# Weepingchestnut/SAVSR

Hardware: AMD Instinct MI355X
Metric: HR Mpixels/sec (Vid4-shape x4, 7-frame window) (higher is better)
Workload: dtype f32 (bf16x3 split products, fp32 accumulate)

## Files before the change

### savsr_amd/csrc/conv_common.hpp

```cpp
#pragma once
#include "common.hpp"

namespace savsr {

struct ConvParams {
    const float* src[SAVSR_MAX_SRC];
    int src_pix[SAVSR_MAX_SRC];
    const unsigned short* wimg;
    const float* bias;
    int act;
    float slope;
    const float* mul_px;
    const float* res1;
    int res1_pix;
    const float* res2;
    int res2_pix;
    float res2_scale;
    float* out;
    int out_pix;
    float* pool;
    int pool_stride;
};

#ifndef SAVSR_CONV_MAX_BATCH
#define SAVSR_CONV_MAX_BATCH 24
#endif
constexpr int CONV_MAX_BATCH = SAVSR_CONV_MAX_BATCH;
constexpr int CONV_WIDE_MIN_TILES = 200;
constexpr int CONV_WIDE_MIN_TILES_TP = 100;
#ifndef SAVSR_CONV_BLOCKS
#define SAVSR_CONV_BLOCKS 256
#endif
constexpr int CONV_PERSISTENT_BLOCKS = SAVSR_CONV_BLOCKS;
#ifndef WY_STRIP
#define WY_STRIP 1
#endif
struct MultiConvParams {
    ConvParams c[CONV_MAX_BATCH];
    int h, w, cout, nchunk, src_ch;
    int nconv, ncob, ntx, nty;
    int wy_tiles, wy_full, wy_strip_l2;
};
static_assert(sizeof(MultiConvParams) <= 4096, "MultiConvParams is passed by value as the conv kernels' argument: at most 4 KB");

int launch_conv_wy(const MultiConvParams& mp, hipStream_t st, bool f16);
int conv_wy_prepare_device();

typedef _Float16 f16x8 __attribute__((ext_vector_type(8)));
typedef _Float16 f16x4 __attribute__((ext_vector_type(4)));

#define SAVSR_GLOBAL __attribute__((address_space(1)))
__device__ __forceinline__ f32x4 ldg4(const float* base, unsigned byte_off) {
    return *(const SAVSR_GLOBAL f32x4*)((const SAVSR_GLOBAL char*)base + byte_off);
}
__device__ __forceinline__ float ldg1(const float* base, unsigned idx) {
    return *((const SAVSR_GLOBAL float*)base + idx);
}
#ifndef CONV_ST
#define CONV_ST 1
#endif
__device__ __forceinline__ void stg4(float* base, unsigned byte_off, const f32x4& v) {
#if CONV_ST == 1
    __builtin_nontemporal_store(v, (SAVSR_GLOBAL f32x4*)((SAVSR_GLOBAL char*)base + byte_off));
#else
    *(SAVSR_GLOBAL f32x4*)((SAVSR_GLOBAL char*)base + byte_off) = v;
#endif
}
__device__ __forceinline__ float vmax_raw(float a, float b) {
    float r;
    asm("v_max_f32 %0, %1, %2" : "=v"(r) : "v"(a), "v"(b));
    return r;
}
__device__ __forceinline__ void stg1(float* base, unsigned idx, float v) {
    *((SAVSR_GLOBAL float*)base + idx) = v;
}

}
```

### savsr_amd/csrc/conv_wy.hip

```cpp
#include "conv_common.hpp"

#include <type_traits>

#ifndef WY_STAMPS
#define WY_STAMPS 0
#endif
#ifndef WY_VALU
#define WY_VALU 6
#endif
#ifndef WY_FAST_EPILOGUE
#define WY_FAST_EPILOGUE 1
#endif
#ifndef WY_BUF
#define WY_BUF 1
#endif

namespace savsr {

namespace wy {
constexpr int TH = 16, TW = 32, NTHR = 512, COT = 64;
[[maybe_unused]] constexpr int IC = TW + 2;
#ifndef WY_ICP
#define WY_ICP 36
#endif
constexpr int ICP = WY_ICP;
constexpr int V_PLANE = 2 * ICP;
constexpr int V_WAVE = 2 * 2 * 2 * V_PLANE;
constexpr int W_HALF = 6 * 2 * 2 * 64;
constexpr int W_PHASE = 2 * W_HALF;
constexpr int EPS = 36;
constexpr int LDS_UNITS = 8 * V_WAVE + 2 * W_HALF;
constexpr size_t LDS_BYTES = 16ull * LDS_UNITS + 4ull * 8 * 32 * EPS;
static_assert(LDS_BYTES <= 160 * 1024, "LDS budget");
}

__device__ __attribute__((aligned(16))) const float g_wy_zero16[4] = {0.f, 0.f, 0.f, 0.f};

#if WY_STAMPS
__device__ long long g_wy_stamps[256 * 8 * 8];
#define WY_KSEC(i) (WY_STAMPS == 2 ? 0 : (i))
#define WY_MARK(i) do { const long long t_now = (long long)__builtin_amdgcn_s_memtime(); wy_sec[i] += t_now - wy_prev; wy_prev = t_now; } while (0)
#if WY_STAMPS == 2
#define WY_EMARK(i) WY_MARK(i)
#endif
#else
#define WY_KSEC(i) (i)
#define WY_MARK(i) do { } while (0)
#endif

typedef float f32x2 __attribute__((ext_vector_type(2)));
typedef __bf16 bf16x2 __attribute__((ext_vector_type(2)));
__device__ __forceinline__ void wy_split_store(const f32x4& v, bf16x4* hi_dst, bf16x4* lo_dst) {
    typedef unsigned u32x2 __attribute__((ext_vector_type(2)));
    const f32x2 a[2] = {{v[0], v[1]}, {v[2], v[3]}};
    u32x2 hi, lo;
#pragma unroll
    for (int p = 0; p < 2; ++p) hi[p] = __builtin_bit_cast(unsigned, __builtin_convertvector(a[p], bf16x2));
    asm("" : "+v"(hi[0]), "+v"(hi[1]));
#pragma unroll
    for (int p = 0; p < 2; ++p) {
        const f32x2 back = {__builtin_bit_cast(float, hi[p] << 16), __builtin_bit_cast(float, hi[p] & 0xffff0000u)};
        const f32x2 rest = {a[p][0] - back[0], a[p][1] - back[1]};
        lo[p] = __builtin_bit_cast(unsigned, __builtin_convertvector(rest, bf16x2));
    }
    *hi_dst = __builtin_bit_cast(bf16x4, hi);
    *lo_dst = __builtin_bit_cast(bf16x4, lo);
}
__device__ __forceinline__ void wy_f16_store(const f32x4& v, bf16x4* hi_dst) {
    f16x4 h;
#pragma unroll
    for (int j = 0; j < 4; ++j) h[j] = (_Float16)v[j];
    *hi_dst = __builtin_bit_cast(bf16x4, h);
}

template <bool FAST, bool F16>
__global__ __launch_bounds__(512) void conv_wy_kernel(const MultiConvParams mp) {
    using namespace wy;
    constexpr int WPH = F16 ? W_PHASE / 2 : W_PHASE, WHF = F16 ? W_HALF / 2 : W_HALF;
    extern __shared__ __attribute__((aligned(16))) unsigned char smem_raw[];
    bf16x8* smem = reinterpret_cast<bf16x8*>(smem_raw);
    const int tid = threadIdx.x, lane = tid & 63, wave = tid >> 6, half = lane >> 5, px = lane & 31;
    const int wave_s = __builtin_amdgcn_readfirstlane(wave);
    const int tiles_per_cob = mp.wy_tiles;
    const int total = mp.nconv * mp.ncob * tiles_per_cob;
    const int H = mp.h, W = mp.w;

    struct TileInfo { int conv, cob, x0, y0, tx, ty, strip; };
    auto decode = [&](int tile) {
        const int cc = (int)((unsigned)tile / (unsigned)tiles_per_cob), rem = tile - cc * tiles_per_cob;
        const bool strip = rem >= mp.wy_full;
        const int tyf = (int)((unsigned)rem / (unsigned)mp.ntx);
        const int l2 = strip ? mp.wy_strip_l2 : 3;
        const int ty = strip ? mp.nty - 1 : tyf;
        const int tx = strip ? (rem - mp.wy_full) << (3 - l2) : rem - tyf * mp.ntx;
        const int wx = tx + (wave_s >> l2);
        TileInfo ti;
        ti.conv = (int)((unsigned)cc / (unsigned)mp.ncob);
        ti.cob = cc - ti.conv * mp.ncob;
        ti.x0 = (wx < mp.ntx ? wx : tx) * TW;
        ti.y0 = wx < mp.ntx ? ty * TH - 2 * ((wave_s >> l2) << l2) : mp.nty * TH;
        ti.tx = tx;
        ti.ty = ty;
        ti.strip = strip ? 1 : 0;
        return ti;
    };

    f32x4 d[2][4], dx;
#if !WY_BUF
    int st_pxb[2], st_pxt;
    constexpr int INVALID = -(1 << 30);
#endif
    const float* st_base = nullptr;
    const bf16x8* st_w = nullptr;
    int st_pix = 0, st_cb = 0, st_src = 0, st_conv = 0, st_row0 = 0;
    const int q4 = lane & 3;
#if WY_BUF
    constexpr unsigned OOB = 0x80000000u;
    unsigned st_vcol[2], st_vtail;
    int st_x0 = 0;
    auto stage_cols = [&]() {
#pragma unroll
        for (int r = 0; r < 2; ++r) {
            const int x = st_x0 - 1 + (lane >> 2) + 16 * r;
            const unsigned v = (unsigned)(x * st_pix + 4 * q4) * 4u;
            st_vcol[r] = (unsigned)x < (unsigned)W ? v : OOB;
        }
        const int x = st_x0 - 1 + 32 + ((lane & 7) >> 2), rr = (lane >> 3) & 3, row = st_row0 + rr;
        const unsigned vt = (unsigned)((rr * W + x) * st_pix + 4 * q4) * 4u;
        const bool okt = (lane < 32) & ((unsigned)x < (unsigned)W) & ((unsigned)row < (unsigned)H);
        st_vtail = okt ? vt : OOB;
    };
#endif
#if WY_BUF
    auto uni = [](int v) { return __builtin_amdgcn_readfirstlane(v); };
    auto uni_ptr = [](const float* q) {
        const unsigned long long a = (unsigned long long)(uintptr_t)q;
        const unsigned lo = (unsigned)__builtin_amdgcn_readfirstlane((int)(unsigned)a), hi = (unsigned)__builtin_amdgcn_readfirstlane((int)(unsigned)(a >> 32));
        return (const float*)(uintptr_t)(((unsigned long long)hi << 32) | lo);
    };
#else
    auto uni = [](int v) { return v; };
    auto uni_ptr = [](const float* q) { return q; };
#endif
    auto stage_begin_tile = [&](const TileInfo& ti) {
        st_conv = ti.conv;
        st_src = 0;
        st_cb = 0;
        st_base = uni_ptr(mp.c[ti.conv].src[0]);
        st_pix = uni(mp.c[ti.conv].src_pix[0]);
        st_w = reinterpret_cast<const bf16x8*>(mp.c[ti.conv].wimg) + (long long)ti.cob * mp.nchunk * WPH;
        st_row0 = uni(ti.y0 + 2 * wave_s - 1);
#if WY_BUF
        st_x0 = ti.x0;
        stage_cols();
#else
#pragma unroll
        for (int r = 0; r < 2; ++r) {
            const int x = ti.x0 - 1 + (lane >> 2) + 16 * r;
            st_pxb[r] = (x >= 0 && x < W) ? st_row0 * W + x : INVALID;
        }
        {
            const int x = ti.x0 - 1 + 32 + ((lane & 7) >> 2), row = st_row0 + ((lane >> 3) & 3);
            st_pxt = (lane < 32 && x >= 0 && x < W && row >= 0 && row < H) ? row * W + x : INVALID;
        }
#endif
    };
    auto stage_advance = [&]() {
        st_cb += 16;
        st_w += WPH;
        if (st_cb >= mp.src_ch) {
            st_cb = 0;
            ++st_src;
            st_base = uni_ptr(mp.c[st_conv].src[st_src]);
#if WY_BUF
            const int pix_new = uni(mp.c[st_conv].src_pix[st_src]);
            if (pix_new != st_pix) { st_pix = pix_new; stage_cols(); }
#else
            st_pix = mp.c[st_conv].src_pix[st_src];
#endif
        }
    };
    int st_tile = blockIdx.x, st_chunk = 0;
    auto stage_next = [&]() -> bool {
        if (st_chunk + 1 < mp.nchunk) { ++st_chunk; stage_advance(); return true; }
        if (st_tile + (int)gridDim.x >= total) return false;
        st_tile += gridDim.x;
        st_chunk = 0;
        stage_begin_tile(decode(st_tile));
        return true;
    };
#if WY_BUF
    typedef unsigned u32x4_t __attribute__((ext_vector_type(4)));
    auto row_rsrc = [&](int i, bool whole) {
        const int off = ((st_row0 + i) * W * st_pix + st_cb) * 4;
        const bool row_ok = whole || (st_row0 + i >= 0 && st_row0 + i < H);
        return __builtin_amdgcn_make_buffer_rsrc((void*)((const char*)st_base + off), (short)0, row_ok ? 0x7fffffff : 0, 0x00020000);
    };
    auto issue_row = [&](int r, int i) {
        d[r][i] = __builtin_bit_cast(f32x4, (u32x4_t)__builtin_amdgcn_raw_buffer_load_b128(row_rsrc(i, false), (int)st_vcol[r], 0, 0));
    };
    auto issue_d = [&](int r) {
#pragma unroll
        for (int i = 0; i < 4; ++i) issue_row(r, i);
    };
    auto issue_dx = [&]() { dx = __builtin_bit_cast(f32x4, (u32x4_t)__builtin_amdgcn_raw_buffer_load_b128(row_rsrc(0, true), (int)st_vtail, 0, 0)); };
#else
    auto load_at = [&](int pixel, bool ok) -> f32x4 {
        const SAVSR_GLOBAL float* src = ok ? (const SAVSR_GLOBAL float*)st_base + (pixel * st_pix + st_cb + 4 * q4)
                                           : (const SAVSR_GLOBAL float*)g_wy_zero16;
        return *(const SAVSR_GLOBAL f32x4*)src;
    };
    auto issue_row = [&](int r, int i) {
        const bool row_ok = st_row0 + i >= 0 && st_row0 + i < H;
        d[r][i] = load_at(st_pxb[r] + i * W, row_ok && st_pxb[r] != INVALID);
    };
    auto issue_d = [&](int r) {
#pragma unroll
        for (int i = 0; i < 4; ++i) issue_row(r, i);
    };
    auto issue_dx = [&]() { dx = load_at(st_pxt, st_pxt != INVALID); };
#endif
    bf16x8* vwave = smem + wave * V_WAVE;
    constexpr int PLANE_B = V_PLANE * 16;
    const unsigned vst0 = (unsigned)(wave * V_WAVE + (q4 >> 1) * ICP + (lane >> 2)) * 16u + (unsigned)(q4 & 1) * 8u;
    const unsigned vst_t = (unsigned)(wave * V_WAVE + (q4 >> 1) * ICP + 32 + ((lane & 7) >> 2)) * 16u + (unsigned)(q4 & 1) * 8u;
    auto vptr = [&](unsigned off) { return reinterpret_cast<bf16x4*>(smem_raw + off); };
    auto vstore = [&](const f32x4& v, unsigned off) {
        if constexpr (F16) wy_f16_store(v, vptr(off));
        else wy_split_store(v, vptr(off), vptr(off + PLANE_B));
    };
    auto store_pair = [&](int r, int hf, const f32x4& va, const f32x4& vb) {
        vstore(va, vst0 + (unsigned)(r * 256 + (hf * 2 + 0) * 2 * PLANE_B));
        vstore(vb, vst0 + (unsigned)(r * 256 + (hf * 2 + 1) * 2 * PLANE_B));
    };
    auto store_one = [&](int r, int hf, int vr, const f32x4& v) {
        vstore(v, vst0 + (unsigned)(r * 256 + (hf * 2 + vr) * 2 * PLANE_B));
    };
    auto store_v0 = [&](int r) { store_one(r, 0, 0, d[r][0] - d[r][2]); };
    auto store_v1 = [&](int r) {
        store_one(r, 0, 1, d[r][1] + d[r][2]);
        const f32x4 v2 = d[r][2] - d[r][1], v3 = d[r][1] - d[r][3];
        d[r][0] = v2;
        d[r][1] = v3;
    };
    auto store_v01 = [&](int r) { store_v0(r); store_v1(r); };
    auto store_v23 = [&](int r) { store_pair(r, 1, d[r][0], d[r][1]); };
    const int grp = (lane >> 3) & 3;
    auto tail_value = [&](int hf) -> f32x4 {
        const int partner = hf == 0 ? (grp == 0 ? lane ^ 16 : lane ^ 24) : (grp == 2 ? lane ^ 24 : lane ^ 16);
        f32x4 o;
#pragma unroll
        for (int j = 0; j < 4; ++j) o[j] = __shfl(dx[j], partner, 64);
        return (hf == 0 && grp == 1) ? dx + o : dx - o;
    };
    auto tail_store = [&](int hf, const f32x4& v) {
        const bool mine = lane < 32 && (hf == 0 ? grp < 2 : (grp == 2 || grp == 1));
        const int vr = hf == 0 ? grp : (grp == 2 ? 0 : 1);
        if (mine) {
            vstore(v, vst_t + (unsigned)((hf * 2 + vr) * 2 * PLANE_B));
        }
    };
    auto store_vt01 = [&]() {
        const f32x4 v01 = tail_value(0), v23 = tail_value(1);
        tail_store(0, v01);
        dx = v23;
    };
    auto store_vt23 = [&]() { tail_store(1, dx); };
    bf16x8* wlds = smem + 8 * V_WAVE;
    [[maybe_unused]] const unsigned lane16 = (unsigned)lane * 16u;
    auto issue_w = [&](int j, int hf) {
        const int piece = F16 ? j * 8 + wave_s : wave_s * 3 + j;
        if (F16 && piece >= 12) return;
        const unsigned dst = __builtin_amdgcn_readfirstlane((unsigned)(uintptr_t)(wlds + hf * W_HALF + piece * (F16 ? 128 : 64)));
        unsigned keep;
#if WY_BUF
        asm volatile("s_mov_b32 %0, m0\n\ts_mov_b32 m0, %3\n\ts_nop 0\n\tglobal_load_lds_dwordx4 %1, %2\n\ts_mov_b32 m0, %0"
                     : "=&s"(keep) : "v"(lane16), "s"(st_w + hf * WHF + piece * 64), "s"(dst) : "memory");
#else
        asm volatile("s_mov_b32 %0, m0\n\ts_mov_b32 m0, %2\n\ts_nop 0\n\tglobal_load_lds_dwordx4 %1, off\n\ts_mov_b32 m0, %0"
                     : "=&s"(keep) : "v"(st_w + hf * WHF + piece * 64 + lane), "s"(dst) : "memory");
#endif
    };

    struct FragA { bf16x8 ah, al; };
    struct FragB { bf16x8 bh, bl; };
    const bf16x8* vrd = vwave + half * ICP + px;
    const bf16x8* wrd = wlds + lane;
    auto load_b = [&](int hf, int s, FragB& fr) {
        const int vr = s / 3, kx = s - 3 * vr;
        fr.bh = vrd[((hf * 2 + vr) * 2 + 0) * V_PLANE + kx];
        if (!F16) fr.bl = vrd[((hf * 2 + vr) * 2 + 1) * V_PLANE + kx];
    };
    auto load_a = [&](int hf, int s, int t, FragA& fr) {
        fr.ah = wrd[hf * W_HALF + ((s * 2 + t) * 2 + 0) * 64];
        if (!F16) fr.al = wrd[hf * W_HALF + ((s * 2 + t) * 2 + 1) * 64];
    };

    int tile = blockIdx.x;
#if WY_STAMPS
    long long wy_sec[8] = {0, 0, 0, 0, 0, 0, 0, 0};
    long long wy_prev = (long long)__builtin_amdgcn_s_memtime();
    const long long wy_t0 = wy_prev;
#endif
    FragA fa[2];
    FragB fb[2];
    if (tile < total) {
        stage_begin_tile(decode(tile));
#pragma unroll
        for (int j = 0; j < 3; ++j) issue_w(j, 0);
        issue_d(0);
        issue_d(1);
        issue_dx();
        store_v01(0);
        store_v01(1);
        store_vt01();
    }
    asm volatile("s_waitcnt vmcnt(0)" ::: "memory");
    __syncthreads();
    if (tile < total) { load_b(0, 0, fb[0]); load_a(0, 0, 0, fa[0]); }

    for (; tile < total; tile += gridDim.x) {
        const TileInfo cur = decode(tile);
        const ConvParams& p = mp.c[cur.conv];
        const int cob = cur.cob, x0 = cur.x0, y0 = cur.y0;
        f32x16 acc[4][2];
#pragma unroll
        for (int pz = 0; pz < 4; ++pz)
#pragma unroll
            for (int t = 0; t < 2; ++t)
#pragma unroll
                for (int i = 0; i < 16; ++i) acc[pz][t][i] = 0.f;
        const bool rows_in = y0 + 2 * wave_s < H;
        for (int chunk = 0; chunk < mp.nchunk; ++chunk) {
            auto phase = [&](auto mm) {
                constexpr bool MM = decltype(mm)::value;
                auto pieces = [&](int hf, int s) {
                    if (hf == 0) {
                        if (s == 0) { issue_w(0, 1); issue_w(1, 1); store_v23(0); }
                        if (s == 1) { issue_w(2, 1); stage_next(); issue_row(0, 0); }
                        if (s == 2) { store_v23(1); issue_row(0, 1); issue_row(0, 2); }
                        if (s == 3) { store_vt23(); issue_row(0, 3); issue_row(1, 0); }
                        if (s == 4) { issue_row(1, 1); issue_row(1, 2); }
                        if (s == 5) issue_row(1, 3);
                    } else {
                        if (s < 3) issue_w(s, 0);
                        if (s == 1) store_v0(0);
                        if (s == 2) store_v1(0);
                        if (s == 3) store_v0(1);
                        if (s == 4) store_v1(1);
                        if (s == 5) store_vt01();
                    }
                };
                auto mma3 = [&](int pz, int t, int sb) {
                    const FragA& a = fa[t];
                    const FragB& b = fb[sb];
                    if (MM && F16) {
                        acc[pz][t] = __builtin_amdgcn_mfma_f32_32x32x16_f16(__builtin_bit_cast(f16x8, a.ah), __builtin_bit_cast(f16x8, b.bh), acc[pz][t], 0, 0, 0);
                    } else if (MM) {
                        acc[pz][t] = __builtin_amdgcn_mfma_f32_32x32x16_bf16(a.al, b.bh, acc[pz][t], 0, 0, 0);
                        acc[pz][t] = __builtin_amdgcn_mfma_f32_32x32x16_bf16(a.ah, b.bl, acc[pz][t], 0, 0, 0);
                        acc[pz][t] = __builtin_amdgcn_mfma_f32_32x32x16_bf16(a.ah, b.bh, acc[pz][t], 0, 0, 0);
                    }
                };
#pragma unroll
                for (int hf = 0; hf < 2; ++hf) {
#pragma unroll
                    for (int s = 0; s < 5; ++s) {
                        const int pz = hf * 2 + s / 3;
                        load_a(hf, s, 1, fa[1]);
                        load_b(hf, s + 1, fb[(s + 1) & 1]);
                        __builtin_amdgcn_sched_barrier(0);
                        mma3(pz, 0, s & 1);
                        pieces(hf, s);
                        load_a(hf, s + 1, 0, fa[0]);
                        mma3(pz, 1, s & 1);
                        if (MM && F16) {
#pragma unroll
                            for (int i = 0; i < 2; ++i) {
                                __builtin_amdgcn_sched_group_barrier(0x008, 1, 0);
                                if (i == 1) __builtin_amdgcn_sched_group_barrier(0x100, 1, 0);
                                __builtin_amdgcn_sched_group_barrier(0x002, 3 * WY_VALU, 0);
                                __builtin_amdgcn_sched_group_barrier(0x200, 2, 0);
                                __builtin_amdgcn_sched_group_barrier(0x010, 1, 0);
                            }
                        } else if (MM) {
#pragma unroll
                            for (int i = 0; i < 6; ++i) {
                                __builtin_amdgcn_sched_group_barrier(0x008, 1, 0);
                                if (i == 3) __builtin_amdgcn_sched_group_barrier(0x100, 2, 0);
                                __builtin_amdgcn_sched_group_barrier(0x002, WY_VALU, 0);
                                __builtin_amdgcn_sched_group_barrier(0x200, 1, 0);
                                if (i == 1 || i == 4) __builtin_amdgcn_sched_group_barrier(0x010, 1, 0);
                            }
                        }
                        __builtin_amdgcn_sched_barrier(0);
                    }
                    {
                        const int pz = hf * 2 + 1;
                        load_a(hf, 5, 1, fa[1]);
                        __builtin_amdgcn_sched_barrier(0);
                        mma3(pz, 0, 1);
                        pieces(hf, 5);
                        if (MM) {
#pragma unroll
                            for (int i = 0; i < (F16 ? 1 : 3); ++i) {
                                __builtin_amdgcn_sched_group_barrier(0x008, 1, 0);
                                __builtin_amdgcn_sched_group_barrier(0x002, 10, 0);
                                __builtin_amdgcn_sched_group_barrier(0x200, 1, 0);
                            }
                        }
                        __builtin_amdgcn_sched_barrier(0);
                        WY_MARK(WY_KSEC(hf * 3 + 0));
                        if (hf == 0) asm volatile("s_waitcnt vmcnt(8)" ::: "memory");
                        else asm volatile("s_waitcnt vmcnt(0)" ::: "memory");
                        __syncthreads();
                        WY_MARK(WY_KSEC(hf * 3 + 1));
                        load_b(hf ^ 1, 0, fb[0]);
                        load_a(hf ^ 1, 0, 0, fa[0]);
                        __builtin_amdgcn_sched_barrier(0);
                        mma3(pz, 1, 1);
                        if (hf == 0) issue_dx();
                        __builtin_amdgcn_sched_barrier(0);
                    }
                    WY_MARK(WY_KSEC(hf * 3 + 2));
                }
            };
            auto phase_dead = [&]() {
#pragma unroll
                for (int j = 0; j < 3; ++j) issue_w(j, 1);
                stage_next();
                asm volatile("s_waitcnt vmcnt(0)" ::: "memory");
                __syncthreads();
#pragma unroll
                for (int j = 0; j < 3; ++j) issue_w(j, 0);
                asm volatile("s_waitcnt vmcnt(0)" ::: "memory");
                __syncthreads();
            };
            auto next_tile_rows_in = [&]() {
                if (tile + (int)gridDim.x >= total) return false;
                return decode(tile + (int)gridDim.x).y0 + 2 * wave_s < H;
            };
            if (rows_in) phase(std::true_type{});
            else if (chunk + 1 == mp.nchunk && next_tile_rows_in()) phase(std::false_type{});
            else phase_dead();
        }

        const float* e_bias = p.bias;
        const float* e_mul = p.mul_px;
        const float* e_r1 = p.res1;
        const float* e_r2 = p.res2;
        float* e_out = p.out;
        float* e_pool = p.pool;
        int e_act = p.act, e_opix = p.out_pix, e_r1pix = p.res1_pix, e_r2pix = p.res2_pix;
        float e_slope = p.slope, e_r2s = p.res2_scale;
        asm volatile("" : "+s"(e_bias), "+s"(e_mul), "+s"(e_r1), "+s"(e_r2), "+s"(e_out), "+s"(e_pool));
        asm volatile("" : "+s"(e_act), "+s"(e_opix), "+s"(e_r1pix), "+s"(e_r2pix), "+s"(e_slope), "+s"(e_r2s));
        const bool act_as_max = e_act == SAVSR_ACT_NONE || e_act == SAVSR_ACT_RELU || (e_act == SAVSR_ACT_LRELU && e_slope >= 0.f && e_slope <= 1.f);
        const float slope_eff = e_act == SAVSR_ACT_NONE ? 1.f : (e_act == SAVSR_ACT_RELU ? 0.f : e_slope);
        float* ep_base = reinterpret_cast<float*>(smem + LDS_UNITS);
        float* ep = ep_base + wave * (32 * EPS);
        const int c4 = lane & 7;
        const bool x_inside = x0 + TW <= W;
        const float* zero16 = (const float*)g_wy_zero16;
        const float* b_base = e_bias ? e_bias : zero16;
        const unsigned b_off = e_bias ? 4u * (unsigned)(cob * COT + 4 * c4) : 0u, b_step = e_bias ? 128u : 0u;
        f32x4 bias4[2];
#pragma unroll
        for (int t = 0; t < 2; ++t) bias4[t] = ldg4(b_base, b_off + (unsigned)t * b_step);
        const float* r1_base = e_r1 ? e_r1 : zero16;
        constexpr int RR = 2;
        f32x4 rr[RR][4];
        auto load_r1 = [&](int r, int t, f32x4 (&dst)[4]) {
            const int y = y0 + 2 * wave_s + r;
            const int co = cob * COT + 32 * t + 4 * c4;
            const unsigned off0 = 4u * (unsigned)((y * W + x0 + (lane >> 3)) * e_r1pix + co), ustride = 32u * (unsigned)e_r1pix;
            const bool row_ok = e_r1 && y < H;
#pragma unroll
            for (int i = 0; i < 4; ++i) {
                const bool ok = row_ok && (x_inside || x0 + (lane >> 3) + 8 * i < W);
                dst[i] = ldg4(r1_base, ok ? off0 + (unsigned)i * ustride : 0u);
            }
        };
#pragma unroll
        for (int gi = 0; gi < RR; ++gi) load_r1(gi / 2, gi % 2, rr[gi]);
        __builtin_amdgcn_sched_barrier(0);
#pragma unroll
        for (int t = 0; t < 2; ++t)
#pragma unroll
            for (int i = 0; i < 16; ++i) {
                const float m1 = acc[1][t][i], m2 = acc[2][t][i];
                acc[0][t][i] = (acc[0][t][i] + m1) + m2;
                acc[3][t][i] = (m1 - m2) - acc[3][t][i];
            }
        f32x4 psum[2][2];
#ifdef WY_EMARK
        asm volatile("" :: "v"(acc[0][0][0]), "v"(acc[3][1][15]));
        WY_EMARK(1);
#endif
#pragma unroll
        for (int r = 0; r < 2; ++r) {
            const int y = y0 + 2 * wave_s + r;
            const int pbase = y * W + x0 + (lane >> 3);
#pragma unroll
            for (int t = 0; t < 2; ++t) {
                psum[r][t] = f32x4{0.f, 0.f, 0.f, 0.f};
                const int gi = r * 2 + t;
                if (y >= H) {
                    asm volatile("" :: "v"(bias4[t]), "v"(rr[gi % RR][0]), "v"(rr[gi % RR][1]), "v"(rr[gi % RR][2]), "v"(rr[gi % RR][3]));
                    if (gi + RR < 4) load_r1((gi + RR) / 2, (gi + RR) % 2, rr[gi % RR]);
                    continue;
                }
                const f32x16& a = r == 0 ? acc[0][t] : acc[3][t];
#pragma unroll
                for (int g = 0; g < 4; ++g) {
                    const f32x4 v = {a[4 * g], a[4 * g + 1], a[4 * g + 2], a[4 * g + 3]};
                    *reinterpret_cast<f32x4*>(ep + px * EPS + 8 * g + 4 * half) = v;
                }
                const int co = cob * COT + 32 * t + 4 * c4;
                const f32x4 b4 = bias4[t];
                const unsigned ooff0 = 4u * (unsigned)(pbase * e_opix + co), ostride = 32u * (unsigned)e_opix;
                f32x4 ps = {0.f, 0.f, 0.f, 0.f};
#pragma unroll
                for (int ih = 0; ih < 2; ++ih) {
                    const int p0 = pbase + 16 * ih;
                    const bool ok0 = x_inside || x0 + (lane >> 3) + 16 * ih < W, ok1 = x_inside || x0 + (lane >> 3) + 16 * ih + 8 < W;
                    f32x4 v[2];
#pragma unroll
                    for (int i = 0; i < 2; ++i) {
                        const f32x4 a4 = *reinterpret_cast<const f32x4*>(ep + ((lane >> 3) + 16 * ih + 8 * i) * EPS + 4 * c4);
                        v[i] = a4 + b4;
                    }
                    if constexpr (FAST) {
#pragma unroll
                        for (int i = 0; i < 2; ++i) {
                            const f32x4 sv = v[i] * slope_eff;
#pragma unroll
                            for (int q = 0; q < 4; ++q) v[i][q] = vmax_raw(v[i][q], sv[q]);
                        }
                    } else if (e_act == SAVSR_ACT_NONE) {
                    } else if (act_as_max) {
#pragma unroll
                        for (int i = 0; i < 2; ++i) {
                            const f32x4 sv = v[i] * slope_eff;
#pragma unroll
                            for (int q = 0; q < 4; ++q) v[i][q] = vmax_raw(v[i][q], sv[q]);
                        }
                    } else if (e_act == SAVSR_ACT_LRELU) {
#pragma unroll
                        for (int i = 0; i < 2; ++i)
#pragma unroll
                            for (int q = 0; q < 4; ++q) v[i][q] = v[i][q] > 0.f ? v[i][q] : v[i][q] * e_slope;
                    } else if (e_act == SAVSR_ACT_SIGMOID) {
#pragma unroll
                        for (int i = 0; i < 2; ++i)
#pragma unroll
                            for (int q = 0; q < 4; ++q) v[i][q] = sigmoidf_(v[i][q]);
                    }
                    if (!FAST && e_mul) {
                        const float m0 = ok0 ? ldg1(e_mul, (unsigned)p0) : 0.f, m1 = ok1 ? ldg1(e_mul, (unsigned)(p0 + 8)) : 0.f;
#pragma unroll
                        for (int q = 0; q < 4; ++q) { v[0][q] *= m0; v[1][q] *= m1; }
                    }
                    v[0] += rr[gi % RR][2 * ih];
                    v[1] += rr[gi % RR][2 * ih + 1];
                    if (!FAST && e_r2) {
                        f32x4 ra = {0.f, 0.f, 0.f, 0.f}, rb = {0.f, 0.f, 0.f, 0.f};
                        if (ok0) ra = ldg4(e_r2, 4u * (unsigned)(p0 * e_r2pix + co));
                        if (ok1) rb = ldg4(e_r2, 4u * (unsigned)((p0 + 8) * e_r2pix + co));
#pragma unroll
                        for (int q = 0; q < 4; ++q) { v[0][q] += e_r2s * ra[q]; v[1][q] += e_r2s * rb[q]; }
                    }
#pragma unroll
                    for (int i = 0; i < 2; ++i) {
                        if (i == 0 ? ok0 : ok1) {
                            stg4(e_out, ooff0 + (unsigned)(2 * ih + i) * ostride, v[i]);
                            if (e_pool) ps += v[i];
                        }
                    }
                }
                psum[r][t] = ps;
#ifdef WY_EMARK
                WY_EMARK(2 + gi);
#endif
                if (gi + RR < 4) load_r1((gi + RR) / 2, (gi + RR) % 2, rr[gi % RR]);
            }
        }
        if (e_pool) {
#pragma unroll
            for (int r = 0; r < 2; ++r)
#pragma unroll
                for (int t = 0; t < 2; ++t)
#pragma unroll
                    for (int o = 8; o < 64; o <<= 1) {
                        psum[r][t][0] += __shfl_xor(psum[r][t][0], o, 64); psum[r][t][1] += __shfl_xor(psum[r][t][1], o, 64);
                        psum[r][t][2] += __shfl_xor(psum[r][t][2], o, 64); psum[r][t][3] += __shfl_xor(psum[r][t][3], o, 64);
                    }
            __syncthreads();
            float* pl_ = ep_base;
            if (lane < 8)
#pragma unroll
                for (int r = 0; r < 2; ++r)
#pragma unroll
                    for (int t = 0; t < 2; ++t) *reinterpret_cast<f32x4*>(pl_ + (wave * 2 + r) * COT + 32 * t + 4 * lane) = psum[r][t];
            __syncthreads();
            const TileInfo pt = decode(tile);
            const int l2p = pt.strip ? mp.wy_strip_l2 : 2;
            if (tid < (8 >> l2p) * COT) {
                const int sg = tid / COT, ch = tid - sg * COT;
                float sacc = 0.f;
#pragma unroll
                for (int k = 0; k < 8; ++k)
                    if (k < (2 << l2p)) sacc += pl_[(((sg << l2p) * 2) + k) * COT + ch];
                const int band = pt.ty * 2 + (pt.strip ? 0 : sg), ptx = pt.tx + (pt.strip ? sg : 0);
                if (band * 8 < H && ptx < mp.ntx) stg1(e_pool, (unsigned)((band * mp.ntx + ptx) * p.pool_stride + cob * COT + ch), sacc);
            }
            __syncthreads();
        }
        WY_MARK(6);
    }
#if WY_STAMPS
    wy_sec[7] = (long long)__builtin_amdgcn_s_memtime() - wy_t0;
    if (lane == 0 && blockIdx.x < 256)
        for (int i = 0; i < 8; ++i) g_wy_stamps[(blockIdx.x * 8 + wave) * 8 + i] = wy_sec[i];
#endif
    asm volatile("s_waitcnt vmcnt(0)" ::: "memory");
}

int launch_conv_wy(const MultiConvParams& mp, hipStream_t st, bool f16) {
    if (int rc = conv_wy_prepare_device()) return rc;
    const int total = mp.nconv * mp.ncob * mp.wy_tiles;
    const int grid = total < CONV_PERSISTENT_BLOCKS ? total : CONV_PERSISTENT_BLOCKS;
    bool fast = WY_FAST_EPILOGUE != 0;
    for (int i = 0; i < mp.nconv && fast; ++i) {
        const ConvParams& c = mp.c[i];
        const bool as_max = c.act == SAVSR_ACT_NONE || c.act == SAVSR_ACT_RELU || (c.act == SAVSR_ACT_LRELU && c.slope >= 0.f && c.slope <= 1.f);
        fast = as_max && !c.mul_px && !c.res2;
    }
    if (f16) {
        if (fast) hipLaunchKernelGGL((conv_wy_kernel<true, true>), dim3(grid), dim3(wy::NTHR), wy::LDS_BYTES, st, mp);
        else hipLaunchKernelGGL((conv_wy_kernel<false, true>), dim3(grid), dim3(wy::NTHR), wy::LDS_BYTES, st, mp);
    } else if (fast) hipLaunchKernelGGL((conv_wy_kernel<true, false>), dim3(grid), dim3(wy::NTHR), wy::LDS_BYTES, st, mp);
    else hipLaunchKernelGGL((conv_wy_kernel<false, false>), dim3(grid), dim3(wy::NTHR), wy::LDS_BYTES, st, mp);
    return check_launch("conv_wy_kernel");
}
int conv_wy_prepare_device() {
    if (int rc = ensure_dynamic_lds(reinterpret_cast<const void*>(&conv_wy_kernel<true, false>), (int)wy::LDS_BYTES, "conv_wy")) return rc;
    if (int rc = ensure_dynamic_lds(reinterpret_cast<const void*>(&conv_wy_kernel<false, false>), (int)wy::LDS_BYTES, "conv_wy")) return rc;
    if (int rc = ensure_dynamic_lds(reinterpret_cast<const void*>(&conv_wy_kernel<true, true>), (int)wy::LDS_BYTES, "conv_wy")) return rc;
    return ensure_dynamic_lds(reinterpret_cast<const void*>(&conv_wy_kernel<false, true>), (int)wy::LDS_BYTES, "conv_wy");
}

}

using namespace savsr;

#if WY_STAMPS
extern "C" int savsr_debug_read_wy_stamps(long long* host) {
    return (int)hipMemcpyFromSymbol(host, HIP_SYMBOL(g_wy_stamps), sizeof(long long) * 256 * 8 * 8);
}
#endif

extern "C" int64_t savsr_conv_wy_packed_elems(int cout, int cin) {
    if (cout <= 0 || cout % 64 || cin <= 0 || cin % 16) return -1;
    return (int64_t)(cout / 64) * (cin / 16) * 12 * 16 * 64;
}
extern "C" int64_t savsr_conv_wy_pack_index(int cout, int cin, int co, int ci, int pos, int kx) {
    const int64_t nchunk = cin / 16;
    const int cob = co / 64, col = co % 64, t = col / 32, row = col % 32;
    const int chunk = ci / 16, cl = ci % 16, kh = cl / 8, j = cl % 8;
    const int hf = pos / 2, vr = pos % 2, s = vr * 3 + kx;
    const int64_t group = ((((int64_t)(cob * nchunk + chunk) * 2 + hf) * 6 + s) * 2 + t);
    return group * 512 + (kh * 32 + row) * 8 + j;
}
```

Measured before the change: 142.5.

## Use buffer-resource loads/stores with hardware bounds checks in Winograd conv epilogue

Replaces per-lane bounds predicates and zero-pointer fallbacks in the conv epilogue with raw buffer loads and stores whose resource descriptors encode the valid range, so out-of-range lanes are handled by hardware clamping. It also precomputes the per-wave LDS destination for weight prefetch so m0 is set with a single scalar add, skips the activation max when the activation is none, and caches the tile key for pooling instead of decoding the tile again. The cost is building several buffer descriptors per slice, plus a new host check that pixel strides are at least cout.

```diff
diff --git a/savsr_amd/csrc/conv_common.hpp b/savsr_amd/csrc/conv_common.hpp
--- a/savsr_amd/csrc/conv_common.hpp
+++ b/savsr_amd/csrc/conv_common.hpp
@@ -66,6 +66,10 @@
     *(SAVSR_GLOBAL f32x4*)((SAVSR_GLOBAL char*)base + byte_off) = v;
 #endif
 }
+__device__ __forceinline__ void bstg4(__amdgpu_buffer_rsrc_t rs, int byte_off, const f32x4& v) {
+    typedef unsigned u32x4s __attribute__((ext_vector_type(4)));
+    __builtin_amdgcn_raw_buffer_store_b128(__builtin_bit_cast(u32x4s, v), rs, byte_off, 0, CONV_ST == 1 ? 2 : 0);
+}
 __device__ __forceinline__ float vmax_raw(float a, float b) {
     float r;
     asm("v_max_f32 %0, %1, %2" : "=v"(r) : "v"(a), "v"(b));
diff --git a/savsr_amd/csrc/conv_wy.hip b/savsr_amd/csrc/conv_wy.hip
--- a/savsr_amd/csrc/conv_wy.hip
+++ b/savsr_amd/csrc/conv_wy.hip
@@ -34,7 +34,7 @@
 static_assert(LDS_BYTES <= 160 * 1024, "LDS budget");
 }
 
-__device__ __attribute__((aligned(16))) const float g_wy_zero16[4] = {0.f, 0.f, 0.f, 0.f};
+[[maybe_unused]] __device__ __attribute__((aligned(16))) const float g_wy_zero16[4] = {0.f, 0.f, 0.f, 0.f};
 
 #if WY_STAMPS
 __device__ long long g_wy_stamps[256 * 8 * 8];
@@ -84,6 +84,7 @@
     const int tiles_per_cob = mp.wy_tiles;
     const int total = mp.nconv * mp.ncob * tiles_per_cob;
     const int H = mp.h, W = mp.w;
+    __builtin_assume(mp.nchunk > 0);
 
     struct TileInfo { int conv, cob, x0, y0, tx, ty, strip; };
     auto decode = [&](int tile) {
@@ -268,17 +269,24 @@
     auto store_vt23 = [&]() { tail_store(1, dx); };
     bf16x8* wlds = smem + 8 * V_WAVE;
     [[maybe_unused]] const unsigned lane16 = (unsigned)lane * 16u;
+    const unsigned wdst_wave = __builtin_amdgcn_readfirstlane((unsigned)(uintptr_t)(wlds + wave_s * (F16 ? 128 : 3 * 64)));
     auto issue_w = [&](int j, int hf) {
         const int piece = F16 ? j * 8 + wave_s : wave_s * 3 + j;
         if (F16 && piece >= 12) return;
-        const unsigned dst = __builtin_amdgcn_readfirstlane((unsigned)(uintptr_t)(wlds + hf * W_HALF + piece * (F16 ? 128 : 64)));
+        const int dst_imm = (hf * W_HALF + j * (F16 ? 8 * 128 : 64)) * 16;
         unsigned keep;
 #if WY_BUF
+#ifdef WY_X_OLDM0
+        const unsigned dst_x = __builtin_amdgcn_readfirstlane((unsigned)(uintptr_t)(wlds + hf * W_HALF + piece * (F16 ? 128 : 64)));
         asm volatile("s_mov_b32 %0, m0\n\ts_mov_b32 m0, %3\n\ts_nop 0\n\tglobal_load_lds_dwordx4 %1, %2\n\ts_mov_b32 m0, %0"
-                     : "=&s"(keep) : "v"(lane16), "s"(st_w + hf * WHF + piece * 64), "s"(dst) : "memory");
-#else
-        asm volatile("s_mov_b32 %0, m0\n\ts_mov_b32 m0, %2\n\ts_nop 0\n\tglobal_load_lds_dwordx4 %1, off\n\ts_mov_b32 m0, %0"
-                     : "=&s"(keep) : "v"(st_w + hf * WHF + piece * 64 + lane), "s"(dst) : "memory");
+                     : "=&s"(keep) : "v"(lane16), "s"(st_w + hf * WHF + piece * 64), "s"(dst_x) : "memory");
+#else
+        asm volatile("s_mov_b32 %0, m0\n\ts_add_u32 m0, %3, %4\n\ts_nop 0\n\tglobal_load_lds_dwordx4 %1, %2\n\ts_mov_b32 m0, %0"
+                     : "=&s"(keep) : "v"(lane16), "s"(st_w + hf * WHF + piece * 64), "s"(wdst_wave), "i"(dst_imm) : "memory", "scc");
+#endif
+#else
+        asm volatile("s_mov_b32 %0, m0\n\ts_add_u32 m0, %2, %3\n\ts_nop 0\n\tglobal_load_lds_dwordx4 %1, off\n\ts_mov_b32 m0, %0"
+                     : "=&s"(keep) : "v"(st_w + hf * WHF + piece * 64 + lane), "s"(wdst_wave), "i"(dst_imm) : "memory", "scc");
 #endif
     };
 
@@ -323,6 +331,7 @@
         const TileInfo cur = decode(tile);
         const ConvParams& p = mp.c[cur.conv];
         const int cob = cur.cob, x0 = cur.x0, y0 = cur.y0;
+        const int pool_key = __builtin_amdgcn_readfirstlane((cur.ty << 17) | (cur.tx << 1) | cur.strip);
         f32x16 acc[4][2];
 #pragma unroll
         for (int pz = 0; pz < 4; ++pz)
@@ -459,27 +468,40 @@
         const float slope_eff = e_act == SAVSR_ACT_NONE ? 1.f : (e_act == SAVSR_ACT_RELU ? 0.f : e_slope);
         float* ep_base = reinterpret_cast<float*>(smem + LDS_UNITS);
         float* ep = ep_base + wave * (32 * EPS);
-        const int c4 = lane & 7;
-        const bool x_inside = x0 + TW <= W;
-        const float* zero16 = (const float*)g_wy_zero16;
-        const float* b_base = e_bias ? e_bias : zero16;
-        const unsigned b_off = e_bias ? 4u * (unsigned)(cob * COT + 4 * c4) : 0u, b_step = e_bias ? 128u : 0u;
+        const int c4 = lane & 7, lpx = lane >> 3;
+        const int n_in = W - x0 < TW ? W - x0 : TW;
+        auto slice_rsrc = [&](const float* base, int pix, int y, int k) {
+            const int off = ((y * W + x0 + 8 * k) * pix + cob * COT) * 4;
+            const int n_eff = (base != nullptr && y < H) ? n_in : 0;
+            const int nrec = n_eff > 8 * k ? (n_eff - 1 - 8 * k) * pix * 4 + COT * 4 : 0;
+            return __builtin_amdgcn_make_buffer_rsrc((void*)((const char*)base + off), (short)0, nrec, 0x00020000);
+        };
+        [[maybe_unused]] auto mask_rsrc = [&](int y, int k) {
+            const int left = y < H ? n_in - 8 * k : 0;
+            return __builtin_amdgcn_make_buffer_rsrc((void*)(e_mul + (y * W + x0 + 8 * k)), (short)0, left > 0 ? 4 * left : 0, 0x00020000);
+        };
+        typedef unsigned eu32x4 __attribute__((ext_vector_type(4)));
         f32x4 bias4[2];
-#pragma unroll
-        for (int t = 0; t < 2; ++t) bias4[t] = ldg4(b_base, b_off + (unsigned)t * b_step);
-        const float* r1_base = e_r1 ? e_r1 : zero16;
+        {
+            const auto b_rs = __builtin_amdgcn_make_buffer_rsrc((void*)(e_bias + cob * COT), (short)0, e_bias ? COT * 4 : 0, 0x00020000);
+#pragma unroll
+            for (int t = 0; t < 2; ++t) bias4[t] = __builtin_bit_cast(f32x4, (eu32x4)__builtin_amdgcn_raw_buffer_load_b128(b_rs, 16 * c4 + 128 * t, 0, 0));
+        }
         constexpr int RR = 2;
         f32x4 rr[RR][4];
+        const int r1_voff = (lpx * e_r1pix + 4 * c4) * 4, o_voff = (lpx * e_opix + 4 * c4) * 4;
         auto load_r1 = [&](int r, int t, f32x4 (&dst)[4]) {
             const int y = y0 + 2 * wave_s + r;
-            const int co = cob * COT + 32 * t + 4 * c4;
-            const unsigned off0 = 4u * (unsigned)((y * W + x0 + (lane >> 3)) * e_r1pix + co), ustride = 32u * (unsigned)e_r1pix;
-            const bool row_ok = e_r1 && y < H;
-#pragma unroll
-            for (int i = 0; i < 4; ++i) {
-                const bool ok = row_ok && (x_inside || x0 + (lane >> 3) + 8 * i < W);
-                dst[i] = ldg4(r1_base, ok ? off0 + (unsigned)i * ustride : 0u);
+#pragma unroll
+            for (int i = 0; i < 4; ++i)
+#ifdef WY_X_FLATLD
+            {
+                const bool ok = e_r1 && y < H && lpx < n_in - 8 * i;
+                dst[i] = ldg4(e_r1 ? e_r1 : (const float*)g_wy_zero16, ok ? 4u * (unsigned)((y * W + x0 + 8 * i) * e_r1pix + cob * COT) + (unsigned)(r1_voff + 128 * t) : 0u);
             }
+#else
+                dst[i] = __builtin_bit_cast(f32x4, (eu32x4)__builtin_amdgcn_raw_buffer_load_b128(slice_rsrc(e_r1, e_r1pix, y, i), r1_voff + 128 * t, 0, 0));
+#endif
         };
 #pragma unroll
         for (int gi = 0; gi < RR; ++gi) load_r1(gi / 2, gi % 2, rr[gi]);
@@ -500,7 +522,6 @@
 #pragma unroll
         for (int r = 0; r < 2; ++r) {
             const int y = y0 + 2 * wave_s + r;
-            const int pbase = y * W + x0 + (lane >> 3);
 #pragma unroll
             for (int t = 0; t < 2; ++t) {
                 psum[r][t] = f32x4{0.f, 0.f, 0.f, 0.f};
@@ -516,14 +537,10 @@
                     const f32x4 v = {a[4 * g], a[4 * g + 1], a[4 * g + 2], a[4 * g + 3]};
                     *reinterpret_cast<f32x4*>(ep + px * EPS + 8 * g + 4 * half) = v;
                 }
-                const int co = cob * COT + 32 * t + 4 * c4;
                 const f32x4 b4 = bias4[t];
-                const unsigned ooff0 = 4u * (unsigned)(pbase * e_opix + co), ostride = 32u * (unsigned)e_opix;
                 f32x4 ps = {0.f, 0.f, 0.f, 0.f};
 #pragma unroll
                 for (int ih = 0; ih < 2; ++ih) {
-                    const int p0 = pbase + 16 * ih;
-                    const bool ok0 = x_inside || x0 + (lane >> 3) + 16 * ih < W, ok1 = x_inside || x0 + (lane >> 3) + 16 * ih + 8 < W;
                     f32x4 v[2];
 #pragma unroll
                     for (int i = 0; i < 2; ++i) {
@@ -531,12 +548,15 @@
                         v[i] = a4 + b4;
                     }
                     if constexpr (FAST) {
-#pragma unroll
-                        for (int i = 0; i < 2; ++i) {
-                            const f32x4 sv = v[i] * slope_eff;
-#pragma unroll
-                            for (int q = 0; q < 4; ++q) v[i][q] = vmax_raw(v[i][q], sv[q]);
-                        }
+#if !defined(WY_X_NOSKIP)
+                        if (e_act != SAVSR_ACT_NONE)
+#endif
+#pragma unroll
+                            for (int i = 0; i < 2; ++i) {
+                                const f32x4 sv = v[i] * slope_eff;
+#pragma unroll
+                                for (int q = 0; q < 4; ++q) v[i][q] = vmax_raw(v[i][q], sv[q]);
+                            }
                     } else if (e_act == SAVSR_ACT_NONE) {
                     } else if (act_as_max) {
 #pragma unroll
@@ -557,25 +577,31 @@
                             for (int q = 0; q < 4; ++q) v[i][q] = sigmoidf_(v[i][q]);
                     }
                     if (!FAST && e_mul) {
-                        const float m0 = ok0 ? ldg1(e_mul, (unsigned)p0) : 0.f, m1 = ok1 ? ldg1(e_mul, (unsigned)(p0 + 8)) : 0.f;
-#pragma unroll
-                        for (int q = 0; q < 4; ++q) { v[0][q] *= m0; v[1][q] *= m1; }
+                        float m[2];
+#pragma unroll
+                        for (int i = 0; i < 2; ++i) m[i] = __builtin_bit_cast(float, __builtin_amdgcn_raw_buffer_load_b32(mask_rsrc(y, 2 * ih + i), 4 * lpx, 0, 0));
+#pragma unroll
+                        for (int q = 0; q < 4; ++q) { v[0][q] *= m[0]; v[1][q] *= m[1]; }
                     }
                     v[0] += rr[gi % RR][2 * ih];
                     v[1] += rr[gi % RR][2 * ih + 1];
                     if (!FAST && e_r2) {
-                        f32x4 ra = {0.f, 0.f, 0.f, 0.f}, rb = {0.f, 0.f, 0.f, 0.f};
-                        if (ok0) ra = ldg4(e_r2, 4u * (unsigned)(p0 * e_r2pix + co));
-                        if (ok1) rb = ldg4(e_r2, 4u * (unsigned)((p0 + 8) * e_r2pix + co));
-#pragma unroll
-                        for (int q = 0; q < 4; ++q) { v[0][q] += e_r2s * ra[q]; v[1][q] += e_r2s * rb[q]; }
+                        const int r2_voff = (lpx * e_r2pix + 4 * c4) * 4;
+                        f32x4 r2v[2];
+#pragma unroll
+                        for (int i = 0; i < 2; ++i)
+                            r2v[i] = __builtin_bit_cast(f32x4, (eu32x4)__builtin_amdgcn_raw_buffer_load_b128(slice_rsrc(e_r2, e_r2pix, y, 2 * ih + i), r2_voff + 128 * t, 0, 0));
+#pragma unroll
+                        for (int q = 0; q < 4; ++q) { v[0][q] += e_r2s * r2v[0][q]; v[1][q] += e_r2s * r2v[1][q]; }
                     }
 #pragma unroll
                     for (int i = 0; i < 2; ++i) {
-                        if (i == 0 ? ok0 : ok1) {
-                            stg4(e_out, ooff0 + (unsigned)(2 * ih + i) * ostride, v[i]);
-                            if (e_pool) ps += v[i];
-                        }
+#ifdef WY_X_FLATST
+                        if (lpx < n_in - 8 * (2 * ih + i)) stg4(e_out, 4u * (unsigned)((y * W + x0 + 8 * (2 * ih + i)) * e_opix + cob * COT) + (unsigned)(o_voff + 128 * t), v[i]);
+#else
+                        bstg4(slice_rsrc(e_out, e_opix, y, 2 * ih + i), o_voff + 128 * t, v[i]);
+#endif
+                        if (e_pool && lpx < n_in - 8 * (2 * ih + i)) ps += v[i];
                     }
                 }
                 psum[r][t] = ps;
@@ -597,13 +623,15 @@
                     }
             __syncthreads();
             float* pl_ = ep_base;
-            if (lane < 8)
+            int pl_lane = lane;
+            asm volatile("" : "+v"(pl_lane));
+            if (pl_lane < 8)
 #pragma unroll
                 for (int r = 0; r < 2; ++r)
 #pragma unroll
                     for (int t = 0; t < 2; ++t) *reinterpret_cast<f32x4*>(pl_ + (wave * 2 + r) * COT + 32 * t + 4 * lane) = psum[r][t];
             __syncthreads();
-            const TileInfo pt = decode(tile);
+            struct { int tx, ty, strip; } pt = {(pool_key >> 1) & 0xffff, pool_key >> 17, pool_key & 1};
             const int l2p = pt.strip ? mp.wy_strip_l2 : 2;
             if (tid < (8 >> l2p) * COT) {
                 const int sg = tid / COT, ch = tid - sg * COT;
@@ -628,6 +656,11 @@
 
 int launch_conv_wy(const MultiConvParams& mp, hipStream_t st, bool f16) {
     if (int rc = conv_wy_prepare_device()) return rc;
+    for (int i = 0; i < mp.nconv; ++i) {
+        const ConvParams& c = mp.c[i];
+        if (c.out_pix < mp.cout || (c.res1 && c.res1_pix < mp.cout) || (c.res2 && c.res2_pix < mp.cout))
+            return fail_arg("conv (Winograd-y): the pixel strides of out / res1 / res2 must be at least cout");
+    }
     const int total = mp.nconv * mp.ncob * mp.wy_tiles;
     const int grid = total < CONV_PERSISTENT_BLOCKS ? total : CONV_PERSISTENT_BLOCKS;
     bool fast = WY_FAST_EPILOGUE != 0;
```

After: 141.7. Within noise of the previous version (-0.6%).
